# lastz/lastz

Measured on AMD Instinct MI355X. Metric: Gbp-of-target aligned/sec (whole job, --nogapped HSP path, both strands), higher is better.
Workload: dtype s32

## Files before the change

lastz_amd/csrc/lz_ctx.hpp:

```cpp
#pragma once
#include <hip/hip_runtime.h>
#include <string>
#include <vector>
#include <map>
#include <mutex>
#include "lz_common.hpp"
#include "../../include/lzgpu.h"

struct DevBuf {
    void*  p = nullptr;
    size_t cap = 0;
    int ensure(size_t bytes);
    void release();
    template <class T> T* as() const { return (T*)p; }
};

struct KernelTimer {
    struct Pending { int id; hipEvent_t a, b; hipStream_t s; };
    bool enabled = false;
    std::vector<std::string> names;
    std::vector<uint64_t> launches;
    std::vector<double> ms;
    std::vector<Pending> pending;
    std::map<hipStream_t, std::vector<hipEvent_t>> pool;
// ... 31 lines not shown
    bool inited = false;
    int  device = -1;
    int  num_cus = 256;
    hipStream_t stream = nullptr;
    hipStream_t stream2 = nullptr, stream3 = nullptr;
    hipStream_t dp_stream = nullptr;
    hipEvent_t ev_keys[LZ_SETS] = {}, ev_summ[LZ_SETS] = {}, ev_part[LZ_SETS] = {}, ev_extended[LZ_SETS] = {}, ev_init = nullptr;
    std::string last_error;

    SeqSlot target;
    bool have_table = false;
    lz_table_geom geom;
    LzSeedDev seed;
    DevBuf wstart, wpos;
    u64 num_words = 0;

    std::map<int, SeqSlot> queries;
#define LZ_TEMP_SLOT_B3 (-1000)
    std::mutex slots_m;

    DevBuf cnt, off, pk;
    DevBuf wiv, wsk, wsv;
    DevBuf blk_start;
    std::vector<u64> blk_start_host;
    u32 blk_shift = 0, blk_count = 1;
    u64* pinned = nullptr; size_t pinned_words = 0;
    DevBuf bins[LZ_SETS];
    DevBuf keys[LZ_SETS];
    DevBuf recs[LZ_SETS], bin_base[LZ_SETS];
    DevBuf hist[LZ_SETS], hist_part[LZ_SETS];
// ... 37 lines not shown
int lzk_sample_offsets(LzCtx& c, const u64* off, const u32* cnt, u32 n, u32 stride, u32 ns, u64* out);
int lzk_fill_hits(LzCtx& c, u32 lo, u32 i0, u32 i1, const u32* sk, const u32* sv, u32 n, const u64* off, u64 base, u64* keys, hipStream_t st);
int lzk_hsp_match_counts(LzCtx& c, const LzHspRec* recs, const u32* n_rec_dev, u32 cap, u32 launch_for,
                         const u8* traw, const u8* qraw, const u8* tcode, const u8* qcode, u32* counts, hipStream_t s);
struct LzLutParams; struct LzLutEntry;
#ifndef LZ_PP_TILE_HOST
#define LZ_PP_TILE_HOST 16384
#endif
int lzk_pack2(LzCtx& c, const u8* code_base, const u8* raw_base, u32 len, u8* two, u8* spc, u32 nmask, u32* flags256);
int lzk_overlap32(LzCtx& c, const u8* src, u8* dst, size_t nblocks);
int lzk_hist(LzCtx& c, const u8* bins, u64 n, u32* hist, u32* part, u32* bin_base, hipStream_t st);
int lzk_scan_reserve(LzCtx& c, int set, int mode, u64 max_n);
int lzk_scan_hits(LzCtx& c, int set, int mode, const LzExtendParams& P, const LzLutParams& Q, const u64* keys, u64 n,
                  const s32* score_tab, const LzLutEntry* lut, u8* bins, hipStream_t st);
int lzk_partition(LzCtx& c, int set, const u64* keys, u64 n, const u32* hist, const u32* part, u64* recs, hipStream_t st);
int lzk_settle(LzCtx& c, const LzExtendParams& P, const u64* recs, const u32* bin_base, u32* diag_end,
               const s32* score_tab, LzHspRec* out, u32* out_count, u32 out_cap, u64* counters, hipStream_t s);
```

lastz_amd/csrc/lz_lut.hpp:

```cpp
#pragma once
#include "lz_common.hpp"

#define LZ_PAD2         128
#define LZ_LUT_ENTRIES  4096
#define LZ_LUT_TOTAL    (2 * LZ_LUT_ENTRIES)
#define LZ_LUT_WIN_G    15
#define LZ_LUT_WIN_B    60
#define LZ_LUT_MAXWIN   3
#define LZ_GRAY(c)      ((c) ^ ((c) >> 1))

struct alignas(8) LzLutEntry { u32 ab; u32 sc; };

struct LzLutParams {
    const u8* t2; const u8* q2;
    const u8* tsp; const u8* qsp;
    const u8* t2x; const u8* tspx;
    const u8* tcode; const u8* qcode;
    s32 xdrop;
};

struct LzLutScan { u32 s; s32 run, best; u32 room, used, alive, nwin; };

#if defined(__HIP_DEVICE_COMPILE__)
LZ_HD u32 lz_alignbit(u32 hi, u32 lo, u32 sh) { return __builtin_amdgcn_alignbit(hi, lo, sh); }
// ... 187 lines not shown
{
    s32 diag; LzLutScan L, R;
    lz_lut_init(key, tlen, qlen, diag, L, R);
    while (L.alive == 1 && L.nwin < (u32)LZ_LUT_MAXWIN) lz_lut_step<false, SPECIAL>(P, lut, diag, L, ctab);
    while (R.alive == 1 && R.nwin < (u32)LZ_LUT_MAXWIN) lz_lut_step<true, SPECIAL>(P, lut, diag, R, ctab);
    return lz_lut_summary(L, R, min_score);
}

LZ_HD u64 lz_hit_record(u64 key, u32 summ)
{
    const u32 pos2 = (u32)key, diag = (u32)(key >> 32);
    const bool slow = (summ & LZ_SUMM_SLOW) != 0;
    const u64 payload = slow ? (u64)(diag >> 16) : (u64)(summ & 0xFFFFu);
    return (u64)pos2 | ((u64)(diag & 0xFFu) << 31) | (payload << 39) | (slow ? (1ull << 63) : 0ull);
}
#define LZ_REC_POS2(r)    ((u32)((r) & 0x7FFFFFFFu))
#define LZ_REC_LOW8(r)    ((u32)((r) >> 31) & 0xFFu)
#define LZ_REC_PAYLOAD(r) ((u32)((r) >> 39) & 0xFFFFu)
#define LZ_REC_SLOW(r)    ((u32)((r) >> 63))
LZ_HD u64 lz_rec_with_index(u64 r, u32 idx)
{ return (r & ~((0xFFull << 31) | (0x1Full << 55))) | ((u64)(idx & 0xFFu) << 31) | ((u64)((idx >> 8) & 0x1Fu) << 55); }
#define LZ_REC_INDEX(r)   (((u32)((r) >> 31) & 0xFFu) | (((u32)((r) >> 55) & 0x1Fu) << 8))

template <class Emit>
LZ_HD void lz_settle_record(const LzExtendParams& P, const s32* score_tab, u64 rec, u32 h ,
                            u32& dend, u64& n_ext, u64& n_bp, Emit&& emit)
{
    const u32 p2 = LZ_REC_POS2(rec);
    if (dend > p2 - P.seed_len) return;
    n_ext++;
// ... 12 lines not shown
```

lastz_amd/csrc/lzgpu_api.hip:

```cpp
#include <hip/hip_runtime.h>
#include <stdarg.h>
#include <stdio.h>
#include <stdlib.h>
#include <string.h>
#include <math.h>
#include <algorithm>
#include <mutex>
#include <thread>
#include <atomic>
#include "lz_ctx.hpp"
#include "lz_host.hpp"
#include "lz_lut.hpp"


static LzCtx g_ctx;
static void lz_release_statics();
void lz_phase_clocks_print();
LzCtx& lz_ctx() { return g_ctx; }

static thread_local std::string t_last_error, t_last_error_out;
static std::mutex g_err_m;
int lz_fail(int code, const char* fmt, ...)
{
    char buf[512];
// ... 163 lines not shown

extern "C" void lzgpu_shutdown(void)
{
    LzCtx& c = g_ctx;
    if (!c.inited) return;
    (void)hipSetDevice(c.device);
    (void)hipStreamSynchronize(c.stream);
    lz_phase_clocks_print();
    if (c.stream2) (void)hipStreamSynchronize(c.stream2);
    if (c.stream3) (void)hipStreamSynchronize(c.stream3);
    if (c.dp_stream) (void)hipStreamSynchronize(c.dp_stream);
    c.timer.resolve(); c.dp_timer.resolve();
    if (c.pinned) { (void)hipHostFree(c.pinned); c.pinned = nullptr; c.pinned_words = 0; }
    DevBuf* bufs[] = { &c.target.raw, &c.target.code, &c.wstart, &c.wpos, &c.cnt, &c.off, &c.pk, &c.wiv, &c.wsk, &c.wsv, &c.lut,
                       &c.sort_tmp, &c.scan_tmp, &c.diag_end, &c.score_tab, &c.hsp_out, &c.hsp_count, &c.hsp_mc,
                       &c.dev_counters, &c.tb_keys, &c.tb_vals, &c.tb_keys2, &c.tb_vals2 };
    for (DevBuf* b : bufs) b->release();
    for (int k = 0; k < LZ_SETS; k++) { DevBuf* sb[] = { &c.bins[k], &c.keys[k], &c.recs[k], &c.bin_base[k], &c.hist[k], &c.hist_part[k], &c.summ[k], &c.scan_tasks[k], &c.scan_ntasks[k] }; for (DevBuf* b : sb) b->release(); }
    for (auto& kv : c.queries) { kv.second.raw.release(); kv.second.code.release(); kv.second.dp.release(); kv.second.nib.release(); kv.second.two.release(); kv.second.spc.release(); kv.second.occ_dev.release(); }
    c.target.dp.release(); c.target.nib.release(); c.target.two.release(); c.target.spc.release(); c.target.occ_dev.release();
    c.target.two_x.release(); c.target.spc_x.release();
    lz_release_statics();
    c.queries.clear();
    (void)hipStreamDestroy(c.stream);
    if (c.stream2) (void)hipStreamDestroy(c.stream2);
    if (c.stream3) (void)hipStreamDestroy(c.stream3);
    if (c.dp_stream) (void)hipStreamDestroy(c.dp_stream);
    c.dp_stream = nullptr;
    for (int k = 0; k < LZ_SETS; k++) {
        hipEvent_t* ev[] = { &c.ev_keys[k], &c.ev_summ[k], &c.ev_part[k], &c.ev_extended[k] };
        for (hipEvent_t* e : ev) { if (*e) (void)hipEventDestroy(*e); *e = nullptr; }
    }
    if (c.ev_init) (void)hipEventDestroy(c.ev_init);
    c.ev_init = nullptr; c.stream2 = nullptr; c.stream3 = nullptr;
    c.stream = nullptr; c.inited = false; c.have_table = false; c.device = -1;
    c.n_owners = 1; c.owner = 0; c.last_order.clear();
}

extern "C" void lzgpu_free(void* p) { free(p); }


static int slot_upload(LzCtx& c, SeqSlot& s, const u8* bytes, u32 len, bool keep_host, hipStream_t st = nullptr)
{
    int rc;
    if (!st) st = c.stream;
    size_t total = (size_t)len + 2 * LZ_SEQ_PAD + 16;
    if ((rc = s.raw.ensure(total))) return rc;
    if ((rc = s.code.ensure(total))) return rc;
    LZ_HIP(hipMemsetAsync(s.raw.p, 0, total, st));
    LZ_HIP(hipMemsetAsync(s.code.p, LZ_CODE_INVALID, total, st));
// ... 156 lines not shown
    return rc;
}

extern "C" int lzgpu_table_geom(lz_table_geom* out)
{
    if (!g_ctx.have_table || !out) return lz_fail(LZGPU_ERR_STATE, "no position table");
    *out = g_ctx.geom; return 0;
}

extern "C" int lzgpu_table_adopt(const lz_table_geom* g)
{
    int rc = require_init(); if (rc) return rc;
    LzCtx& c = g_ctx;
    if (!g) return LZGPU_ERR_ARG;
    if ((rc = lzh_seed_to_dev(&g->seed, c.seed))) return rc;
    c.have_table = false; c.geom = *g; c.num_words = g->num_words;
    size_t total = (size_t)g->tlen + 2 * LZ_SEQ_PAD + 16;
    if ((rc = c.target.raw.ensure(total))) return rc;
    if ((rc = c.target.code.ensure(total))) return rc;
    LZ_HIP(hipMemsetAsync(c.target.raw.p, 0, total, c.stream));
    LZ_HIP(hipMemsetAsync(c.target.code.p, LZ_CODE_INVALID, total, c.stream));
    c.target.len = g->tlen; c.target.have_raw = true; c.target.code_key = 0; c.target.dp_key = 0; c.target.host.clear();
    if ((rc = c.wstart.ensure(((size_t)(1u << c.seed.weight) + 1) * 4))) return rc;
    if ((rc = c.wpos.ensure((size_t)(g->num_words ? g->num_words : 1) * 4))) return rc;
    LZ_HIP(hipStreamSynchronize(c.stream));
    return 0;
}

extern "C" int lzgpu_table_buffers(void* dev_ptr[3], uint64_t bytes[3])
{
    LzCtx& c = g_ctx;
// ... 2 lines not shown
    dev_ptr[1] = c.wstart.p;          bytes[1] = ((uint64_t)(1u << c.seed.weight) + 1) * 4;
    dev_ptr[2] = c.wpos.p;            bytes[2] = (uint64_t)c.num_words * 4;
    return 0;
}

extern "C" int lzgpu_table_commit(void)
{
    LzCtx& c = g_ctx;
    if (!c.target.have_raw || !c.wstart.p) return lz_fail(LZGPU_ERR_STATE, "no table buffers");
    { int rc = lz_bind_thread(); if (rc) return rc; }
    if (c.target.host.size() != c.geom.tlen) {
        c.target.host.resize(c.geom.tlen);
        if (c.geom.tlen) LZ_HIP(hipMemcpy(c.target.host.data(), c.target.raw_base(), c.geom.tlen, hipMemcpyDeviceToHost));
        c.target.code_key = 0; c.target.dp_key = 0;
    }
    c.have_table = true;
    return 0;
}

extern "C" int lzgpu_device_copy(void* dst, const void* src, uint64_t bytes)
{
    int rc = require_init(); if (rc) return rc;
    if (!bytes) return 0;
    LZ_HIP(hipMemcpyAsync(dst, src, bytes, hipMemcpyDeviceToDevice, g_ctx.stream));
    LZ_HIP(hipStreamSynchronize(g_ctx.stream));
    return 0;
}


#include <chrono>
struct HostProf {
    bool on; double t[16]; const char* names[16] = { nullptr }; int n = 0;
    std::chrono::steady_clock::time_point last;
    HostProf() { on = getenv("LZGPU_HOSTPROF") != nullptr; for (auto& x : t) x = 0; }
    void start() { if (on) last = std::chrono::steady_clock::now(); }
    void lap(int k, const char* name) {
        if (!on) return;
        auto now = std::chrono::steady_clock::now();
        t[k] += std::chrono::duration<double, std::milli>(now - last).count(); names[k] = name; if (k >= n) n = k + 1; last = now;
    }
    ~HostProf() { if (on) for (int k = 0; k < n; k++) if (names[k]) fprintf(stderr, "[lzgpu hostprof] %-28s %10.2f ms total\n", names[k], t[k]); }
};
static HostProf g_hp;

static int seed_search(const lz_search_args* a, lz_hsp** out, uint64_t* n_out)
{
    int rc = require_init(); if (rc) return rc;
    LzCtx& c = g_ctx;
    if (!a || !out || !n_out || !a->sub) return lz_fail(LZGPU_ERR_ARG, "null argument");
    *out = nullptr; *n_out = 0;
    if (!c.have_table) return lz_fail(LZGPU_ERR_STATE, "lzgpu_table_prepare has not been called");

    g_hp.start();
    SeqSlot* qs;
    if (a->query) {
        if (a->qlen >= 0x7FFFFFFFu) return LZGPU_NH_SIZE;
        qs = lz_query_slot(c, -1, true);
        if ((rc = slot_upload(c, *qs, a->query, a->qlen, false))) return rc;
// ... 65 lines not shown

    std::vector<LzChunk> chunks;
    hipError_t fetch_err = hipSuccess;
    auto off_at = [&](u32 i) -> u64 {
        if (i >= n) return total_hits;
        if (i % S == 0) return samp[i / S];
        u64 v = 0;
        hipError_t e = hipMemcpy(&v, c.off.as<u64>() + i, 8, hipMemcpyDeviceToHost);
        if (e != hipSuccess) fetch_err = e;
        return v;
    };
    if ((rc = lzh_plan_chunks(n, c.hit_capacity, S, off_at, chunks))) return rc;
    if (fetch_err != hipSuccess) return lz_fail(LZGPU_ERR_HIP, "prefix fetch failed: %s", hipGetErrorString(fetch_err));

    g_hp.lap(2, "chunk plan");
    u64 max_chunk = 0;
    for (auto& ch : chunks) if (ch.nh > max_chunk) max_chunk = ch.nh;
    static const bool overlap = getenv("LZGPU_OVERLAP") != nullptr && getenv("LZGPU_SERIAL") == nullptr;
    const int nsets = overlap ? (int)std::min<size_t>(chunks.size() ? chunks.size() : 1, LZ_SETS) : 1;
    if (max_chunk) {
        if ((rc = c.keys[0].ensure((size_t)max_chunk * 8))) return rc;
        if ((rc = c.bins[0].ensure((size_t)max_chunk + 64))) return rc;
        if (a->extend) {
            const size_t ntiles = (size_t)((max_chunk + LZ_PP_TILE_HOST - 1) / LZ_PP_TILE_HOST), nblocks = (ntiles + 255) / 256;
            for (int k = 0; k < nsets; k++) {
                if ((rc = c.keys[k].ensure((size_t)max_chunk * 8))) return rc;
                if ((rc = c.bins[k].ensure((size_t)max_chunk + 64))) return rc;
                if ((rc = c.recs[k].ensure((size_t)max_chunk * 8))) return rc;
                if ((rc = c.bin_base[k].ensure(257 * 4))) return rc;
                if ((rc = c.hist[k].ensure(ntiles * 256 * 4))) return rc;
                if ((rc = c.hist_part[k].ensure(nblocks * 256 * 4))) return rc;
            }
        }
    }
    const u32 out_cap = (u32)std::min<u64>(c.hsp_capacity, 0xFFFFFFF0ull);
    if (a->extend && (rc = c.hsp_out.ensure((size_t)out_cap * sizeof(LzHspRec)))) return rc;

    LzExtendParams P;
    P.tcode = c.target.code_base(); P.tlen = c.geom.tlen;
    P.qcode = qs->code_base();      P.qlen = qlen;
    P.xdrop = a->xdrop; P.min_score = a->hsp_threshold; P.seed_len = L;
    P.cls8 = lzh_small_classes(rowc, colc);
    const bool nibs = P.cls8 && c.target.have_nib && qs->have_nib;
    P.tnib = nibs ? c.target.nib.as<u8>() : nullptr; P.qnib = nibs ? qs->nib.as<u8>() : nullptr;

    LzLutParams Q;
    Q.t2 = c.target.two.as<u8>(); Q.q2 = qs->two.as<u8>(); Q.tsp = c.target.spc.as<u8>(); Q.qsp = qs->spc.as<u8>(); Q.xdrop = a->xdrop;
    Q.t2x = c.target.two_x.as<u8>(); Q.tspx = c.target.spc_x.as<u8>();
    Q.tcode = P.tcode; Q.qcode = P.qcode;
    int mode = 2;
    if (a->extend) {
        s32 M4[16];
// ... 2 lines not shown
        if (mode < c.min_scan_mode) mode = c.min_scan_mode;
        if (mode < 2) {
            static std::vector<LzLutEntry> lut_host; static s32 lut_m4[16]; static s32 lut_x = -1;
            if (lut_x != a->xdrop || memcmp(lut_m4, M4, sizeof(M4)) != 0 || !c.lut.p || lut_host.empty()) {
                lut_host.resize(LZ_LUT_TOTAL);
                lzh_lut_build(M4, a->xdrop, lut_host.data());
                if ((rc = c.lut.ensure(lut_host.size() * sizeof(LzLutEntry)))) return rc;
                memcpy(lut_m4, M4, sizeof(M4)); lut_x = a->xdrop;
                LZ_HIP(hipMemcpyAsync(c.lut.p, lut_host.data(), lut_host.size() * sizeof(LzLutEntry), hipMemcpyHostToDevice, c.stream));
                LZ_HIP(hipStreamSynchronize(c.stream));
            }
        }
    }
    c.last_scan_mode = mode;

    std::vector<lz_hsp> plain;
    if (a->extend && max_chunk) for (int k = 0; k < nsets; k++) if ((rc = lzk_scan_reserve(c, k, mode, max_chunk))) return rc;
    LZ_HIP(hipEventRecord(c.ev_init, c.stream));
    LZ_HIP(hipStreamWaitEvent(c.stream2, c.ev_init, 0));
    LZ_HIP(hipStreamWaitEvent(c.stream3, c.ev_init, 0));
    size_t ci = 0;
    const bool serial = !overlap;
    hipStream_t sF = c.stream, sS = serial ? c.stream : c.stream3, sB = serial ? c.stream : c.stream2;
    auto settle = [&](int set) -> int {
        LZ_HIP(hipStreamWaitEvent(sS, c.ev_part[set], 0));
        int r = lzk_settle(c, P, c.recs[set].as<u64>(), c.bin_base[set].as<u32>(), c.diag_end.as<u32>(), c.score_tab.as<s32>(),
                           c.hsp_out.as<LzHspRec>(), c.hsp_count.as<u32>(), out_cap, d_counters, sS);
        if (r) return r;
        LZ_HIP(hipEventRecord(c.ev_extended[set], sS));
        return 0;
    };
    int pending = -1;
    for (auto& ch : chunks) {
        const int set = (int)(ci % (size_t)nsets);
        if (!a->extend) {
            if ((rc = lzk_fill_hits(c, lo, ch.i0, ch.i1, c.wsk.as<u32>(), c.wsv.as<u32>(), n, c.off.as<u64>(), ch.base, c.keys[0].as<u64>(), sF))) return rc;
            std::vector<u64> hk(ch.nh);
            LZ_HIP(hipMemcpyAsync(hk.data(), c.keys[0].p, (size_t)ch.nh * 8, hipMemcpyDeviceToHost, c.stream));
            LZ_HIP(hipStreamSynchronize(c.stream));
            for (u64 k : hk) { u32 p2 = (u32)k; plain.push_back({ p2 + (u32)(k >> 32), p2, L, 0 }); }
            continue;
        }
        const bool reuse = ci >= (size_t)nsets;
        if (reuse && pending == set) { if ((rc = settle(pending))) return rc; pending = -1; }
        if (reuse) LZ_HIP(hipStreamWaitEvent(sF, c.ev_extended[set], 0));
        if ((rc = lzk_fill_hits(c, lo, ch.i0, ch.i1, c.wsk.as<u32>(), c.wsv.as<u32>(), n, c.off.as<u64>(), ch.base, c.keys[set].as<u64>(), sF))) return rc;
        LZ_HIP(hipEventRecord(c.ev_keys[set], sF));
        LZ_HIP(hipStreamWaitEvent(sS, c.ev_keys[set], 0));
        if ((rc = lzk_scan_hits(c, set, mode, P, Q, c.keys[set].as<u64>(), ch.nh, c.score_tab.as<s32>(), c.lut.as<LzLutEntry>(), c.bins[set].as<u8>(), sS))) return rc;
        LZ_HIP(hipEventRecord(c.ev_summ[set], sS));
        LZ_HIP(hipStreamWaitEvent(sB, c.ev_summ[set], 0));
        if ((rc = lzk_hist(c, c.bins[set].as<u8>(), ch.nh, c.hist[set].as<u32>(), c.hist_part[set].as<u32>(), c.bin_base[set].as<u32>(), sB))) return rc;
        if ((rc = lzk_partition(c, set, c.keys[set].as<u64>(), ch.nh, c.hist[set].as<u32>(), c.hist_part[set].as<u32>(), c.recs[set].as<u64>(), sB))) return rc;
        LZ_HIP(hipEventRecord(c.ev_part[set], sB));
        if (pending >= 0) { if ((rc = settle(pending))) return rc; }
        pending = set;
        ci++;
    }
    if (pending >= 0) { if ((rc = settle(pending))) return rc; }
    g_hp.lap(3, "chunk loop launches");
// ... 184 lines not shown
```

lastz_amd/csrc/seed_kernels.hip:

```cpp
#include <hip/hip_runtime.h>
#include <cstring>
#include <cstdio>
#include <rocprim/device/device_radix_sort.hpp>
#include <rocprim/device/device_scan.hpp>
#include <rocprim/iterator/transform_iterator.hpp>
#include "lz_ctx.hpp"
#include "lz_lut.hpp"
#include "lz_coop.hpp"

#define LZ_TPB 256

#if defined(LZ_NO_NT)
#define LZ_NT_LD(p_) (*(p_))
#define LZ_NT_ST(v_, p_) (*(p_) = (v_))
#else
#define LZ_NT_LD(p_) __builtin_nontemporal_load(p_)
#define LZ_NT_ST(v_, p_) __builtin_nontemporal_store((v_), (p_))
#endif
__global__ void __launch_bounds__(LZ_TPB)
k_encode(const u8* __restrict__ raw, u8* __restrict__ code, u32 len, const u8* __restrict__ cls)
{
    __shared__ u8 tab[256];
    tab[threadIdx.x] = cls[threadIdx.x];
    __syncthreads();
// ... 94 lines not shown
                                     c.tb_vals.as<u32>(), c.tb_vals2.as<u32>(), (size_t)n, 0u,
                                     (unsigned)c.seed.weight + 1u, c.stream));
    c.timer.end(c.stream);

    c.timer.begin("k_key_bounds_u32", c.stream);
    hipLaunchKernelGGL(k_key_bounds_u32, dim3((n + 1 + LZ_TPB - 1) / LZ_TPB), dim3(LZ_TPB), 0, c.stream,
                       c.tb_keys2.as<u32>(), n, nwords, c.wstart.as<u32>());
    c.timer.end(c.stream);
    LZ_HIP(hipGetLastError());

    u32 nw = 0;
    LZ_HIP(hipMemcpyAsync(&nw, c.wstart.as<u32>() + nwords, 4, hipMemcpyDeviceToHost, c.stream));
    LZ_HIP(hipStreamSynchronize(c.stream));
    c.timer.resolve();
    c.num_words = nw;
    if ((rc = c.wpos.ensure((size_t)(nw ? nw : 1) * 4))) return rc;
    LZ_HIP(hipMemcpyAsync(c.wpos.p, c.tb_vals2.p, (size_t)nw * 4, hipMemcpyDeviceToDevice, c.stream));
    LZ_HIP(hipStreamSynchronize(c.stream));
    return 0;
}

__global__ void __launch_bounds__(LZ_TPB)
k_table_export(const u32* __restrict__ wstart, const u32* __restrict__ wpos, u32 nwords,
               u32 adj_start, u32 step, u32* __restrict__ last, u32* __restrict__ prev)
{
    u32 w = blockIdx.x * LZ_TPB + threadIdx.x;
    if (w >= nwords) return;
    u32 a = wstart[w], b = wstart[w + 1];
    if (a == b) return;
    if (last) last[w] = (wpos[a] - adj_start) / step;
// ... 913 lines not shown
        else           hipLaunchKernelGGL(k_scan_tasks<1>, dim3(std::min<u32>(n_regions, 4u * (u32)cus)), dim3(LZ_ST_TPB), 0, st, P, Q, lut, score_tab, tasks, ntk, n_regions, task_cap, summ);
        c.timer.end(st);
        LZ_HIP(hipGetLastError());
    }
    return 0;
}

int lzk_partition(LzCtx& c, int set, const u64* keys, u64 n, const u32* hist, const u32* part, u64* recs, hipStream_t st)
{
    if (n == 0) return 0;
    const u32 ntiles = (u32)((n + LZ_PP_TILE - 1) / LZ_PP_TILE);
    c.timer.begin("k_partition", st);
    static const bool ballots = getenv("LZGPU_PARTITION_BALLOTS") != nullptr;
    if (ballots) hipLaunchKernelGGL(k_partition<false>, dim3(ntiles), dim3(LZ_PP_TPB), 0, st, keys, c.summ[set].as<u32>(), n, hist, part, recs);
    else         hipLaunchKernelGGL(k_partition<true>, dim3(ntiles), dim3(LZ_PP_TPB), 0, st, keys, c.summ[set].as<u32>(), n, hist, part, recs);
    c.timer.end(st);
    LZ_HIP(hipGetLastError());
    return 0;
}

__device__ __forceinline__ LzCoopMap lz_coop_shfl_up32(const LzCoopMap& v, int d)
{ LzCoopMap r; r.A = __shfl_up(v.A, d, 32); r.B = __shfl_up(v.B, d, 32); r.C = __shfl_up(v.C, d, 32); return r; }
__device__ LzCoopSide lz_coop_extend_wave(const LzExtendParams& P, const s32* tab, u32 pos1, s32 diag, s32 stopl, s32 stopr, u32 lane)
{
    const s32 X = P.xdrop;
    const bool right = lane >= 32u;
    const u32 hl = lane & 31u;
    const s32 stop = right ? stopr : stopl;
    LzCoopSide out; out.stop_pos = pos1; out.best_pos = pos1; out.best = 0;
    s32 run0 = 0, best0 = 0; u32 s = pos1;
// ... 322 lines not shown
```

Baseline: 0.3442.

## Fuse hit fill with LUT scan and tag records with bin for partition

Adds a fused kernel that expands seed hits and runs the LUT-based ungapped scan in one pass, writing tagged hit records directly instead of first materializing keys and then rescanning them. A per-word target context cache (32 bytes per word) is prebuilt so the scan can load target windows contiguously, and the bin tag is embedded in each record so histogram and partition read it without a separate bins array. The aim is to cut global memory traffic and kernel launches on the nogapped path, at the cost of extra device memory for the word context and a more complex kernel with large shared-memory use.

Result: faster. 0.3894 (median of 6 runs) (+13.1%).

```diff
diff --git a/lastz_amd/csrc/lz_ctx.hpp b/lastz_amd/csrc/lz_ctx.hpp
--- a/lastz_amd/csrc/lz_ctx.hpp
+++ b/lastz_amd/csrc/lz_ctx.hpp
@@ -69,6 +69,9 @@
     LzSeedDev seed;
     DevBuf wstart, wpos;
     u64 num_words = 0;
+    u64 table_gen = 0;
+    DevBuf wctx;
+    u64 wctx_gen = 0; uint64_t wctx_code_key = 0;
 
     std::map<int, SeqSlot> queries;
 #define LZ_TEMP_SLOT_B3 (-1000)
@@ -136,5 +139,11 @@
 int lzk_scan_hits(LzCtx& c, int set, int mode, const LzExtendParams& P, const LzLutParams& Q, const u64* keys, u64 n,
                   const s32* score_tab, const LzLutEntry* lut, u8* bins, hipStream_t st);
 int lzk_partition(LzCtx& c, int set, const u64* keys, u64 n, const u32* hist, const u32* part, u64* recs, hipStream_t st);
+int lzk_wctx_build(LzCtx& c);
+int lzk_fused_reserve(LzCtx& c, int set, u64 max_n);
+int lzk_scan_fused(LzCtx& c, int set, u32 lo, u32 i0, u32 i1, const u32* sk, const u32* sv, u32 n, const u64* off, u64 base, u64 n_hits,
+                   const LzExtendParams& P, const LzLutParams& Q, const LzLutEntry* lut, u64* tagged, hipStream_t st);
+int lzk_hist_tagged(LzCtx& c, const u64* tagged, u64 n, u32* hist, u32* part, u32* bin_base, hipStream_t st);
+int lzk_partition_tagged(LzCtx& c, const u64* tagged, u64 n, const u32* hist, const u32* part, u64* recs, hipStream_t st);
 int lzk_settle(LzCtx& c, const LzExtendParams& P, const u64* recs, const u32* bin_base, u32* diag_end,
                const s32* score_tab, LzHspRec* out, u32* out_count, u32 out_cap, u64* counters, hipStream_t s);
diff --git a/lastz_amd/csrc/lz_lut.hpp b/lastz_amd/csrc/lz_lut.hpp
--- a/lastz_amd/csrc/lz_lut.hpp
+++ b/lastz_amd/csrc/lz_lut.hpp
@@ -225,6 +225,26 @@
     const u64 payload = slow ? (u64)(diag >> 16) : (u64)(summ & 0xFFFFu);
     return (u64)pos2 | ((u64)(diag & 0xFFu) << 31) | (payload << 39) | (slow ? (1ull << 63) : 0ull);
 }
+#define LZ_REC_TAG(r)     ((u32)((r) >> 55) & 0xFFu)
+#define LZ_REC_UNTAG(r)   ((r) & ~(0xFFull << 55))
+LZ_HD u64 lz_hit_record_tagged(u64 key, u32 summ) { return lz_hit_record(key, summ) | ((u64)((u32)(key >> 40) & 0xFFu) << 55); }
+
+#define LZ_WCTX_BYTES 32
+struct alignas(16) LzWctx { u32 w[LZ_WCTX_BYTES / 4]; };
+LZ_HD u32 lz_wctx_first_byte(u32 pos1) { return ((pos1 - 1u + (u32)LZ_PAD2) >> 2) - 15u; }
+LZ_HD u32 lz_wctx_right_offset(u32 pos1) { return ((pos1 + (u32)LZ_PAD2) >> 2) - lz_wctx_first_byte(pos1); }
+LZ_HD LzWctx lz_wctx_make(const u8* two, u32 pos1) { LzWctx e; __builtin_memcpy(&e, two + lz_wctx_first_byte(pos1), LZ_WCTX_BYTES); return e; }
+LZ_HD void lz_wctx_windows(const LzWctx& e, u32 pos1, LzVec16& tl, LzVec16& tr)
+{
+    const bool at16 = lz_wctx_right_offset(pos1) == 16u;
+    LZ_UNROLL_ALL
+    for (int k = 0; k < 4; k++) {
+        tl.w[k] = e.w[k];
+        const u32 at15 = lz_alignbit(e.w[4 + k], e.w[3 + k], 24u);
+        tr.w[k] = at16 ? e.w[4 + k] : at15;
+    }
+}
+
 #define LZ_REC_POS2(r)    ((u32)((r) & 0x7FFFFFFFu))
 #define LZ_REC_LOW8(r)    ((u32)((r) >> 31) & 0xFFu)
 #define LZ_REC_PAYLOAD(r) ((u32)((r) >> 39) & 0xFFFFu)
diff --git a/lastz_amd/csrc/lzgpu_api.hip b/lastz_amd/csrc/lzgpu_api.hip
--- a/lastz_amd/csrc/lzgpu_api.hip
+++ b/lastz_amd/csrc/lzgpu_api.hip
@@ -201,7 +201,7 @@
     if (c.pinned) { (void)hipHostFree(c.pinned); c.pinned = nullptr; c.pinned_words = 0; }
     DevBuf* bufs[] = { &c.target.raw, &c.target.code, &c.wstart, &c.wpos, &c.cnt, &c.off, &c.pk, &c.wiv, &c.wsk, &c.wsv, &c.lut,
                        &c.sort_tmp, &c.scan_tmp, &c.diag_end, &c.score_tab, &c.hsp_out, &c.hsp_count, &c.hsp_mc,
-                       &c.dev_counters, &c.tb_keys, &c.tb_vals, &c.tb_keys2, &c.tb_vals2 };
+                       &c.dev_counters, &c.tb_keys, &c.tb_vals, &c.tb_keys2, &c.tb_vals2, &c.wctx };
     for (DevBuf* b : bufs) b->release();
     for (int k = 0; k < LZ_SETS; k++) { DevBuf* sb[] = { &c.bins[k], &c.keys[k], &c.recs[k], &c.bin_base[k], &c.hist[k], &c.hist_part[k], &c.summ[k], &c.scan_tasks[k], &c.scan_ntasks[k] }; for (DevBuf* b : sb) b->release(); }
     for (auto& kv : c.queries) { kv.second.raw.release(); kv.second.code.release(); kv.second.dp.release(); kv.second.nib.release(); kv.second.two.release(); kv.second.spc.release(); kv.second.occ_dev.release(); }
@@ -221,6 +221,7 @@
     if (c.ev_init) (void)hipEventDestroy(c.ev_init);
     c.ev_init = nullptr; c.stream2 = nullptr; c.stream3 = nullptr;
     c.stream = nullptr; c.inited = false; c.have_table = false; c.device = -1;
+    c.wctx_gen = 0; c.wctx_code_key = 0;
     c.n_owners = 1; c.owner = 0; c.last_order.clear();
 }
 
@@ -407,7 +408,7 @@
     LzCtx& c = g_ctx;
     if (!g) return LZGPU_ERR_ARG;
     if ((rc = lzh_seed_to_dev(&g->seed, c.seed))) return rc;
-    c.have_table = false; c.geom = *g; c.num_words = g->num_words;
+    c.have_table = false; c.geom = *g; c.num_words = g->num_words; c.table_gen++;
     size_t total = (size_t)g->tlen + 2 * LZ_SEQ_PAD + 16;
     if ((rc = c.target.raw.ensure(total))) return rc;
     if ((rc = c.target.code.ensure(total))) return rc;
@@ -440,6 +441,7 @@
         if (c.geom.tlen) LZ_HIP(hipMemcpy(c.target.host.data(), c.target.raw_base(), c.geom.tlen, hipMemcpyDeviceToHost));
         c.target.code_key = 0; c.target.dp_key = 0;
     }
+    c.table_gen++;
     c.have_table = true;
     return 0;
 }
@@ -468,6 +470,28 @@
     ~HostProf() { if (on) for (int k = 0; k < n; k++) if (names[k]) fprintf(stderr, "[lzgpu hostprof] %-28s %10.2f ms total\n", names[k], t[k]); }
 };
 static HostProf g_hp;
+
+
+static int lz_wctx_prepare(LzCtx& c, bool& fused)
+{
+    if (c.wctx.p && c.wctx_gen == c.table_gen && c.wctx_code_key == c.target.code_key && c.target.code_key) return 0;
+    const size_t need = (size_t)c.num_words * LZ_WCTX_BYTES;
+    if (c.num_words == 0) { fused = false; return 0; }
+    if (need > c.wctx.cap || !c.wctx.p) {
+        size_t fr = 0, tot = 0;
+        if (hipMemGetInfo(&fr, &tot) != hipSuccess || need > (fr + c.wctx.cap) / 2 || c.wctx.ensure(need) != 0) {
+            (void)hipGetLastError(); c.last_error.clear();
+            c.wctx_gen = 0; c.wctx_code_key = 0;
+            fused = false;
+            return 0;
+        }
+    }
+    c.wctx_gen = 0; c.wctx_code_key = 0;
+    int rc = lzk_wctx_build(c);
+    if (rc) return rc;
+    c.wctx_gen = c.table_gen; c.wctx_code_key = c.target.code_key;
+    return 0;
+}
 
 static int seed_search(const lz_search_args* a, lz_hsp** out, uint64_t* n_out)
 {
@@ -563,28 +587,6 @@
     if (fetch_err != hipSuccess) return lz_fail(LZGPU_ERR_HIP, "prefix fetch failed: %s", hipGetErrorString(fetch_err));
 
     g_hp.lap(2, "chunk plan");
-    u64 max_chunk = 0;
-    for (auto& ch : chunks) if (ch.nh > max_chunk) max_chunk = ch.nh;
-    static const bool overlap = getenv("LZGPU_OVERLAP") != nullptr && getenv("LZGPU_SERIAL") == nullptr;
-    const int nsets = overlap ? (int)std::min<size_t>(chunks.size() ? chunks.size() : 1, LZ_SETS) : 1;
-    if (max_chunk) {
-        if ((rc = c.keys[0].ensure((size_t)max_chunk * 8))) return rc;
-        if ((rc = c.bins[0].ensure((size_t)max_chunk + 64))) return rc;
-        if (a->extend) {
-            const size_t ntiles = (size_t)((max_chunk + LZ_PP_TILE_HOST - 1) / LZ_PP_TILE_HOST), nblocks = (ntiles + 255) / 256;
-            for (int k = 0; k < nsets; k++) {
-                if ((rc = c.keys[k].ensure((size_t)max_chunk * 8))) return rc;
-                if ((rc = c.bins[k].ensure((size_t)max_chunk + 64))) return rc;
-                if ((rc = c.recs[k].ensure((size_t)max_chunk * 8))) return rc;
-                if ((rc = c.bin_base[k].ensure(257 * 4))) return rc;
-                if ((rc = c.hist[k].ensure(ntiles * 256 * 4))) return rc;
-                if ((rc = c.hist_part[k].ensure(nblocks * 256 * 4))) return rc;
-            }
-        }
-    }
-    const u32 out_cap = (u32)std::min<u64>(c.hsp_capacity, 0xFFFFFFF0ull);
-    if (a->extend && (rc = c.hsp_out.ensure((size_t)out_cap * sizeof(LzHspRec)))) return rc;
-
     LzExtendParams P;
     P.tcode = c.target.code_base(); P.tlen = c.geom.tlen;
     P.qcode = qs->code_base();      P.qlen = qlen;
@@ -617,8 +619,34 @@
     }
     c.last_scan_mode = mode;
 
+    u64 max_chunk = 0;
+    for (auto& ch : chunks) if (ch.nh > max_chunk) max_chunk = ch.nh;
+    static const bool overlap = getenv("LZGPU_OVERLAP") != nullptr && getenv("LZGPU_SERIAL") == nullptr;
+    const int nsets = overlap ? (int)std::min<size_t>(chunks.size() ? chunks.size() : 1, LZ_SETS) : 1;
+    static const bool fused_off = getenv("LZGPU_FUSED_SCAN") != nullptr && atoi(getenv("LZGPU_FUSED_SCAN")) == 0;
+    bool fused = a->extend && mode == 0 && max_chunk && !fused_off && c.n_owners <= 1 && getenv("LZGPU_FILL_SHUFFLE") == nullptr;
+    if (fused && (rc = lz_wctx_prepare(c, fused))) return rc;
+    if (max_chunk) {
+        if ((rc = c.keys[0].ensure((size_t)max_chunk * 8))) return rc;
+        if (!fused && (rc = c.bins[0].ensure((size_t)max_chunk + 64))) return rc;
+        if (a->extend) {
+            const size_t ntiles = (size_t)((max_chunk + LZ_PP_TILE_HOST - 1) / LZ_PP_TILE_HOST), nblocks = (ntiles + 255) / 256;
+            for (int k = 0; k < nsets; k++) {
+                if ((rc = c.keys[k].ensure((size_t)max_chunk * 8))) return rc;
+                if (!fused && (rc = c.bins[k].ensure((size_t)max_chunk + 64))) return rc;
+                if ((rc = c.recs[k].ensure((size_t)max_chunk * 8))) return rc;
+                if ((rc = c.bin_base[k].ensure(257 * 4))) return rc;
+                if ((rc = c.hist[k].ensure(ntiles * 256 * 4))) return rc;
+                if ((rc = c.hist_part[k].ensure(nblocks * 256 * 4))) return rc;
+            }
+        }
+    }
+    const u32 out_cap = (u32)std::min<u64>(c.hsp_capacity, 0xFFFFFFF0ull);
+    if (a->extend && (rc = c.hsp_out.ensure((size_t)out_cap * sizeof(LzHspRec)))) return rc;
+
+
     std::vector<lz_hsp> plain;
-    if (a->extend && max_chunk) for (int k = 0; k < nsets; k++) if ((rc = lzk_scan_reserve(c, k, mode, max_chunk))) return rc;
+    if (a->extend && max_chunk) for (int k = 0; k < nsets; k++) if ((rc = fused ? lzk_fused_reserve(c, k, max_chunk) : lzk_scan_reserve(c, k, mode, max_chunk))) return rc;
     LZ_HIP(hipEventRecord(c.ev_init, c.stream));
     LZ_HIP(hipStreamWaitEvent(c.stream2, c.ev_init, 0));
     LZ_HIP(hipStreamWaitEvent(c.stream3, c.ev_init, 0));
@@ -647,6 +675,21 @@
         const bool reuse = ci >= (size_t)nsets;
         if (reuse && pending == set) { if ((rc = settle(pending))) return rc; pending = -1; }
         if (reuse) LZ_HIP(hipStreamWaitEvent(sF, c.ev_extended[set], 0));
+        if (fused) {
+            LZ_HIP(hipEventRecord(c.ev_keys[set], sF));
+            LZ_HIP(hipStreamWaitEvent(sS, c.ev_keys[set], 0));
+            if ((rc = lzk_scan_fused(c, set, lo, ch.i0, ch.i1, c.wsk.as<u32>(), c.wsv.as<u32>(), n, c.off.as<u64>(), ch.base, ch.nh, P, Q,
+                                     c.lut.as<LzLutEntry>(), c.keys[set].as<u64>(), sS))) return rc;
+            LZ_HIP(hipEventRecord(c.ev_summ[set], sS));
+            LZ_HIP(hipStreamWaitEvent(sB, c.ev_summ[set], 0));
+            if ((rc = lzk_hist_tagged(c, c.keys[set].as<u64>(), ch.nh, c.hist[set].as<u32>(), c.hist_part[set].as<u32>(), c.bin_base[set].as<u32>(), sB))) return rc;
+            if ((rc = lzk_partition_tagged(c, c.keys[set].as<u64>(), ch.nh, c.hist[set].as<u32>(), c.hist_part[set].as<u32>(), c.recs[set].as<u64>(), sB))) return rc;
+            LZ_HIP(hipEventRecord(c.ev_part[set], sB));
+            if (pending >= 0) { if ((rc = settle(pending))) return rc; }
+            pending = set;
+            ci++;
+            continue;
+        }
         if ((rc = lzk_fill_hits(c, lo, ch.i0, ch.i1, c.wsk.as<u32>(), c.wsv.as<u32>(), n, c.off.as<u64>(), ch.base, c.keys[set].as<u64>(), sF))) return rc;
         LZ_HIP(hipEventRecord(c.ev_keys[set], sF));
         LZ_HIP(hipStreamWaitEvent(sS, c.ev_keys[set], 0));
diff --git a/lastz_amd/csrc/seed_kernels.hip b/lastz_amd/csrc/seed_kernels.hip
--- a/lastz_amd/csrc/seed_kernels.hip
+++ b/lastz_amd/csrc/seed_kernels.hip
@@ -132,6 +132,7 @@
     LZ_HIP(hipStreamSynchronize(c.stream));
     c.timer.resolve();
     c.num_words = nw;
+    c.table_gen++;
     if ((rc = c.wpos.ensure((size_t)(nw ? nw : 1) * 4))) return rc;
     LZ_HIP(hipMemcpyAsync(c.wpos.p, c.tb_vals2.p, (size_t)nw * 4, hipMemcpyDeviceToDevice, c.stream));
     LZ_HIP(hipStreamSynchronize(c.stream));
@@ -1075,6 +1076,334 @@
     static const bool ballots = getenv("LZGPU_PARTITION_BALLOTS") != nullptr;
     if (ballots) hipLaunchKernelGGL(k_partition<false>, dim3(ntiles), dim3(LZ_PP_TPB), 0, st, keys, c.summ[set].as<u32>(), n, hist, part, recs);
     else         hipLaunchKernelGGL(k_partition<true>, dim3(ntiles), dim3(LZ_PP_TPB), 0, st, keys, c.summ[set].as<u32>(), n, hist, part, recs);
+    c.timer.end(st);
+    LZ_HIP(hipGetLastError());
+    return 0;
+}
+
+__global__ void __launch_bounds__(LZ_TPB)
+k_build_wctx(const u32* __restrict__ wpos, u64 num_words, const u8* __restrict__ two, LzVec16* __restrict__ wctx)
+{
+    const u64 j = (u64)blockIdx.x * LZ_TPB + threadIdx.x;
+    if (j >= 2 * num_words) return;
+    const u32 pos1 = wpos[j >> 1];
+    wctx[j] = lz_load16(two + lz_wctx_first_byte(pos1) + 16u * (u32)(j & 1u));
+}
+
+template <int CAP> struct LzFuse2Wave {
+    alignas(16) u32 own32[CAP / 2];
+    u32 lsrc[64 * LZ_FILL_GROUP];
+    uint2 ent[64];
+};
+struct LzFuseTrip { u32 p1, pos2, dst; bool ok; LzWctx cx; LzVec16 ql, qr; };
+
+template <bool SELF, int TPB, int CAP>
+__global__ void __launch_bounds__(TPB)
+k_scan_hits2(u32 lo, u32 i0, u32 i1, LzSeedDev sd,
+             const u32* __restrict__ wstart, const u32* __restrict__ wpos, const LzWctx* __restrict__ wctx,
+             const u32* __restrict__ sk, const u32* __restrict__ sv, u32 n, const u64* __restrict__ off, u64 base,
+             LzExtendParams P, LzLutParams Q, const LzLutEntry* __restrict__ lut_g,
+             u64* __restrict__ recs, LzScanTask* __restrict__ tasks, u32* __restrict__ n_tasks, u32 region_cap, LzSelfDev self)
+{
+    static_assert(CAP % 512 == 0, "whole 16-byte groups of own[] per lane");
+    constexpr int WORDS = CAP / 2 / 64;
+    __shared__ LzLutEntry lut[LZ_LUT_TOTAL];
+    __shared__ LzFuse2Wave<CAP> shw[TPB / 64];
+    for (u32 k = threadIdx.x; k < LZ_LUT_TOTAL; k += TPB) lut[k] = lut_g[k];
+    __syncthreads();
+    LzFuse2Wave<CAP>& sh = shw[threadIdx.x >> 6];
+    unsigned short* const own = reinterpret_cast<unsigned short*>(sh.own32);
+    const u32 lane = threadIdx.x & 63u;
+    const u32 region = blockIdx.x * (TPB / 64) + (threadIdx.x >> 6), nwaves = gridDim.x * (TPB / 64);
+    LzScanTask* const my_tasks = tasks + (size_t)region * region_cap;
+    u32 my_n = 0;
+    const u32 ngroups = (n + 63u) / 64u;
+    for (u32 grp = region; grp < ngroups; grp += nwaves) {
+        const u32 j = grp * 64u + lane;
+        u32 w_l = 0, i_l = 0; bool in = false;
+        if (j < n) { w_l = sk[j] & ((2u << sd.weight) - 1u); i_l = sv[j]; in = !(w_l >> sd.weight) && i_l >= i0 && i_l < i1; }
+        if (!__ballot(in)) continue;
+        const u32 dbase = in ? (u32)(off[i_l] - base) : 0u;
+        const u32 pos2 = lo + i_l + 1u;
+        u32 slo = 0, shi = 0;
+        if (SELF) lz_self_bounds(self, pos2, slo, shi);
+        u32 carry = 0;
+        for (int r = 0; r < sd.nprobes; r += LZ_FILL_GROUP) {
+            u32 la[LZ_FILL_GROUP], len[LZ_FILL_GROUP]; u32 total = 0;
+#pragma unroll
+            for (int p = 0; p < LZ_FILL_GROUP; p++) {
+                const bool on = in && r + p < sd.nprobes;
+                const u32 w = on ? (w_l ^ sd.probe_xor[(r + p) & (LZ_MAX_PROBES - 1)]) : 0u;
+                la[p] = wstart[w]; len[p] = wstart[w + 1];
+            }
+#pragma unroll
+            for (int p = 0; p < LZ_FILL_GROUP; p++) {
+                const bool on = in && r + p < sd.nprobes;
+                len[p] = on ? len[p] - la[p] : 0u;
+                if (!SELF) total += len[p];
+            }
+            if (SELF) {
+                lz_clip_runs<LZ_FILL_GROUP>(wpos, la, len, slo, shi);
+#pragma unroll
+                for (int p = 0; p < LZ_FILL_GROUP; p++) total += len[p];
+            }
+            u32 inc = total;
+            LZ_WAVE_SCAN_U32(inc, total, lz_uadd)
+            const u32 E = inc - total;
+            const u32 T = (u32)__builtin_amdgcn_readlane((int)inc, 63);
+            {
+                u32 S = E;
+#pragma unroll
+                for (int p = 0; p < LZ_FILL_GROUP; p++) { sh.lsrc[lane * LZ_FILL_GROUP + p] = la[p] - S; S += len[p]; }
+            }
+            sh.ent[lane] = make_uint2(dbase + carry - E, pos2);
+            for (u32 cs = 0; cs < T; cs += CAP) {
+                const u32 tc = (T - cs < (u32)CAP) ? T - cs : (u32)CAP;
+                uint4* const mine = reinterpret_cast<uint4*>(sh.own32 + lane * WORDS);
+#pragma unroll
+                for (int k = 0; k < WORDS / 4; k++) mine[k] = make_uint4(0u, 0u, 0u, 0u);
+                __atomic_signal_fence(__ATOMIC_SEQ_CST);
+                {
+                    u32 S = E;
+#pragma unroll
+                    for (int p = 0; p < LZ_FILL_GROUP; p++) {
+                        const u32 l = len[p];
+                        if (l && S < cs + tc && S + l > cs) own[(S > cs ? S : cs) - cs] = (unsigned short)(1u + lane * LZ_FILL_GROUP + (u32)p);
+                        S += l;
+                    }
+                }
+                __atomic_signal_fence(__ATOMIC_SEQ_CST);
+                u32 wv[WORDS];
+#pragma unroll
+                for (int k = 0; k < WORDS / 4; k++) { const uint4 v = mine[k]; wv[4 * k] = v.x; wv[4 * k + 1] = v.y; wv[4 * k + 2] = v.z; wv[4 * k + 3] = v.w; }
+                u32 segmax = 0;
+#pragma unroll
+                for (int k = 0; k < WORDS; k++) { const u32 m2 = lz_umax(wv[k] & 0xFFFFu, wv[k] >> 16); segmax = lz_umax(segmax, m2); }
+                u32 sinc = segmax;
+                LZ_WAVE_SCAN_U32(sinc, segmax, lz_umax)
+                u32 run = lz_dpp_u32<0x138, 0xf, 0xf>(0u, sinc);
+#pragma unroll
+                for (int k = 0; k < WORDS; k++) {
+                    const u32 a0 = lz_umax(wv[k] & 0xFFFFu, run), a1 = lz_umax(wv[k] >> 16, a0);
+                    wv[k] = a0 | (a1 << 16); run = a1;
+                }
+#pragma unroll
+                for (int k = 0; k < WORDS / 4; k++) mine[k] = make_uint4(wv[4 * k], wv[4 * k + 1], wv[4 * k + 2], wv[4 * k + 3]);
+                __atomic_signal_fence(__ATOMIC_SEQ_CST);
+                auto load_trip = [&](u32 tb, LzFuseTrip& t) {
+                    const u32 t0 = tb + lane;
+                    t.ok = t0 < tc;
+                    const u32 tt = t.ok ? t0 : tc - 1u;
+                    const u32 list = (u32)own[tt] - 1u;
+                    const u32 ls = sh.lsrc[list];
+                    const uint2 en = sh.ent[list / LZ_FILL_GROUP];
+                    const u32 tabs = cs + tt, e = ls + tabs;
+                    t.p1 = wpos[e]; t.cx = wctx[e];
+                    t.pos2 = en.y; t.dst = en.x + tabs;
+                    const u32 sql = en.y - 1u + (u32)LZ_PAD2;
+                    t.ql = lz_load16(Q.q2 + ((sql >> 2) - 15u)); t.qr = lz_load16(Q.q2 + ((sql + 1u) >> 2));
+                };
+                auto scan_trip = [&](const LzFuseTrip& t) {
+                    const u64 key = lz_hit_key(t.p1, t.pos2);
+                    LzLutRaw<false> rl, rr;
+                    lz_wctx_windows(t.cx, t.p1, rl.tv, rr.tv);
+                    rl.qv = t.ql; rr.qv = t.qr;
+                    u32 summ;
+                    lz_scan_round<false>(P, Q, lut, nullptr, key, t.ok, rl, rr, t.dst, lane, summ, my_tasks, my_n, region_cap);
+                    if (t.ok) LZ_NT_ST(lz_hit_record_tagged(key, summ), recs + t.dst);
+                };
+                LzFuseTrip ta, tb2;
+                load_trip(0u, ta);
+#pragma unroll 1
+                for (u32 tb = 0;;) {
+                    if (tb + 64u < tc) load_trip(tb + 64u, tb2);
+                    scan_trip(ta);
+                    tb += 64u; if (tb >= tc) break;
+                    if (tb + 64u < tc) load_trip(tb + 64u, ta);
+                    scan_trip(tb2);
+                    tb += 64u; if (tb >= tc) break;
+                }
+                __atomic_signal_fence(__ATOMIC_SEQ_CST);
+            }
+            carry += total;
+        }
+    }
+    if (lane == 0) n_tasks[region] = my_n < region_cap ? my_n : region_cap;
+}
+
+__global__ void __launch_bounds__(LZ_ST_TPB)
+k_scan_tasks2(LzExtendParams P, LzLutParams Q, const LzLutEntry* __restrict__ lut_g, const LzScanTask* __restrict__ tasks,
+              const u32* __restrict__ n_tasks, u32 n_regions, u32 region_cap, u64* __restrict__ recs)
+{
+    __shared__ LzLutEntry lut[LZ_LUT_TOTAL];
+    for (u32 k = threadIdx.x; k < LZ_LUT_TOTAL; k += LZ_ST_TPB) lut[k] = lut_g[k];
+    __syncthreads();
+    for (u32 region = blockIdx.x; region < n_regions; region += gridDim.x) {
+        const u32 nt = n_tasks[region];
+        for (u32 k = threadIdx.x; k < nt; k += (u32)LZ_ST_TPB) {
+            const LzScanTask t = tasks[(size_t)region * region_cap + k];
+            LzLutScan L = t.L, R = t.R;
+            const u32 pos1 = L.alive == 1 ? L.s + (u32)LZ_LUT_WIN_B * L.nwin : R.s - (u32)LZ_LUT_WIN_B * R.nwin;
+            while (L.alive == 1 && L.nwin < (u32)LZ_LUT_MAXWIN) lz_lut_step<false, false>(Q, lut, t.diag, L, nullptr);
+            while (R.alive == 1 && R.nwin < (u32)LZ_LUT_MAXWIN) lz_lut_step<true, false>(Q, lut, t.diag, R, nullptr);
+            recs[t.idx] = lz_hit_record_tagged(lz_hit_key(pos1, pos1 - (u32)t.diag), lz_lut_summary(L, R, P.min_score));
+        }
+    }
+}
+
+__global__ void __launch_bounds__(LZ_TPB)
+k_hist2(const u64* __restrict__ tagged, u64 n, u32* __restrict__ hist)
+{
+    __shared__ u32 cnt[LZ_NBIN];
+    cnt[threadIdx.x] = 0;
+    __syncthreads();
+    const u64 base = (u64)blockIdx.x * LZ_PP_TILE;
+    typedef u64 lz_u64x2 __attribute__((ext_vector_type(2)));
+#pragma unroll 4
+    for (int r = 0; r < LZ_PP_TILE / (LZ_TPB * 2); r++) {
+        const u64 i = base + ((u64)r * LZ_TPB + threadIdx.x) * 2u;
+        if (i + 1u < n) {
+            const lz_u64x2 v = *reinterpret_cast<const lz_u64x2*>(tagged + i);
+            atomicAdd(&cnt[LZ_REC_TAG(v.x)], 1u); atomicAdd(&cnt[LZ_REC_TAG(v.y)], 1u);
+        } else if (i < n) atomicAdd(&cnt[LZ_REC_TAG(tagged[i])], 1u);
+    }
+    __syncthreads();
+    hist[(size_t)blockIdx.x * LZ_NBIN + threadIdx.x] = cnt[threadIdx.x];
+}
+
+__global__ void __launch_bounds__(LZ_PP_TPB)
+k_partition2(const u64* __restrict__ tagged, u64 n, const u32* __restrict__ hist, const u32* __restrict__ part, u64* __restrict__ recs)
+{
+    __shared__ LzPartShared sh;
+    const u32 tid = threadIdx.x, lane = tid & 63u, w = tid >> 6;
+    const u32 tile = blockIdx.x;
+    const u64 base = (u64)tile * LZ_PP_TILE;
+    const u32 tile_n = (n - base < (u64)LZ_PP_TILE) ? (u32)(n - base) : (u32)LZ_PP_TILE;
+    for (u32 k = tid; k < LZ_PP_WAVES * LZ_NBIN; k += LZ_PP_TPB) { (&sh.wcnt[0][0])[k] = 0; (&sh.bm[0][0])[k] = 0ull; }
+    const u32 l0 = w * (64u * LZ_PP_ROUNDS) + lane;
+    u64 rr[LZ_PP_ROUNDS];
+#pragma unroll
+    for (u32 r = 0; r < LZ_PP_ROUNDS; r++) rr[r] = (l0 + 64u * r < tile_n) ? tagged[base + l0 + 64u * r] : 0ull;
+    __syncthreads();
+    u32 slot[LZ_PP_ROUNDS];
+#pragma unroll
+    for (u32 r = 0; r < LZ_PP_ROUNDS; r++) {
+        const bool valid = l0 + 64u * r < tile_n;
+        const u32 bin = LZ_REC_TAG(rr[r]);
+        if (valid) atomicOr((unsigned long long*)&sh.bm[w][bin], 1ull << lane);
+        const u64 peers = valid ? sh.bm[w][bin] : 0ull;
+        const u32 old = valid ? sh.wcnt[w][bin] : 0u;
+        if (valid && (peers >> lane) == 1ull) { sh.wcnt[w][bin] = old + (u32)__popcll(peers); sh.bm[w][bin] = 0ull; }
+        slot[r] = old + (u32)__popcll(peers & ((1ull << lane) - 1ull));
+    }
+    __syncthreads();
+    u32 tot = 0;
+    if (tid < LZ_NBIN) {
+        for (u32 k = 0; k < LZ_PP_WAVES; k++) { const u32 v = sh.wcnt[k][tid]; sh.wcnt[k][tid] = tot; tot += v; }
+        sh.gbase[tid] = part[(size_t)(tile >> 8) * LZ_NBIN + tid] + hist[(size_t)tile * LZ_NBIN + tid];
+    }
+    const u32 ts = lz_exscan256(tot, sh.wtot);
+    if (tid < LZ_NBIN) sh.tstart[tid] = ts;
+    if (tid == 0) sh.tstart[LZ_NBIN] = tile_n;
+    __syncthreads();
+#pragma unroll
+    for (u32 r = 0; r < LZ_PP_ROUNDS; r++) {
+        const u32 bin = LZ_REC_TAG(rr[r]);
+        if (l0 + 64u * r < tile_n) sh.stage[sh.tstart[bin] + sh.wcnt[w][bin] + slot[r]] = rr[r];
+    }
+    __syncthreads();
+    for (u32 k = tid; k < tile_n; k += LZ_PP_TPB) {
+        const u64 r = sh.stage[k];
+        const u32 b = LZ_REC_TAG(r);
+        recs[(size_t)sh.gbase[b] + (k - sh.tstart[b])] = LZ_REC_UNTAG(r);
+    }
+}
+
+int lzk_wctx_build(LzCtx& c)
+{
+    const u64 nw = c.num_words;
+    if (nw == 0) return 0;
+    c.timer.begin("k_build_wctx", c.stream);
+    hipLaunchKernelGGL(k_build_wctx, dim3((unsigned)((2 * nw + LZ_TPB - 1) / LZ_TPB)), dim3(LZ_TPB), 0, c.stream,
+                       c.wpos.as<u32>(), nw, c.target.two.as<u8>(), c.wctx.as<LzVec16>());
+    c.timer.end(c.stream);
+    LZ_HIP(hipGetLastError());
+    return 0;
+}
+
+static u32 lz_fused_tpb(LzCtx& c)
+{
+    static const int env = getenv("LZGPU_FUSE_TPB") ? atoi(getenv("LZGPU_FUSE_TPB")) : 0;
+    if (c.self.mode != LZ_SELF_OFF) return 512u;
+    return (env == 512 || env == 768 || env == 1024) ? (u32)env : 1024u;
+}
+static void lz_fused_geometry(LzCtx& c, u64 n_hits, u32& grid, u32& n_regions, u32& region_cap)
+{
+    int cus = 256; (void)hipDeviceGetAttribute(&cus, hipDeviceAttributeMultiprocessorCount, c.device);
+    grid = (u32)cus; n_regions = grid * (lz_fused_tpb(c) / 64u);
+    region_cap = (u32)std::min<u64>(n_hits / 32 / n_regions + 64, 1u << 20);
+    static const char* force = getenv("LZGPU_TASK_REGION_CAP");
+    if (force && atoi(force) > 0) region_cap = (u32)atoi(force);
+}
+int lzk_fused_reserve(LzCtx& c, int set, u64 max_n)
+{
+    u32 grid, n_regions, region_cap; int rc;
+    lz_fused_geometry(c, max_n, grid, n_regions, region_cap);
+    if ((rc = c.scan_tasks[set].ensure((size_t)n_regions * region_cap * sizeof(LzScanTask)))) return rc;
+    return c.scan_ntasks[set].ensure((size_t)n_regions * 4);
+}
+int lzk_scan_fused(LzCtx& c, int set, u32 lo, u32 i0, u32 i1, const u32* sk, const u32* sv, u32 n, const u64* off, u64 base, u64 n_hits,
+                   const LzExtendParams& P, const LzLutParams& Q, const LzLutEntry* lut, u64* tagged, hipStream_t st)
+{
+    if (n == 0 || i1 <= i0 || n_hits == 0) return 0;
+    if (!c.blk_start_host.empty()) {
+        const u32 b0 = i0 >> c.blk_shift, b1 = (i1 - 1) >> c.blk_shift;
+        const u64 j0 = c.blk_start_host[b0], j1 = c.blk_start_host[std::min<u32>(b1 + 1, c.blk_count)];
+        sk += j0; sv += j0; n = (u32)(j1 - j0);
+        if (n == 0) return 0;
+    }
+    int rc;
+    u32 grid, n_regions, region_cap;
+    lz_fused_geometry(c, n_hits, grid, n_regions, region_cap);
+    if ((rc = c.scan_tasks[set].ensure((size_t)n_regions * region_cap * sizeof(LzScanTask)))) return rc;
+    if ((rc = c.scan_ntasks[set].ensure((size_t)n_regions * 4))) return rc;
+    LzScanTask* tasks = c.scan_tasks[set].as<LzScanTask>(); u32* ntk = c.scan_ntasks[set].as<u32>();
+    c.timer.begin("k_scan_hits", st);
+    const u32 tpb = lz_fused_tpb(c);
+#define LZ_FUSED_LAUNCH(S_, T_, C_, self_) hipLaunchKernelGGL((k_scan_hits2<S_, T_, C_>), dim3(grid), dim3(T_), 0, st, lo, i0, i1, c.seed, c.wstart.as<u32>(), c.wpos.as<u32>(), \
+                           c.wctx.as<LzWctx>(), sk, sv, n, off, base, P, Q, lut, tagged, tasks, ntk, region_cap, self_)
+    if (c.self.mode != LZ_SELF_OFF) LZ_FUSED_LAUNCH(true, 512, 2560, c.self);
+    else if (tpb == 512)            LZ_FUSED_LAUNCH(false, 512, 2560, LzSelfDev{});
+    else if (tpb == 768)            LZ_FUSED_LAUNCH(false, 768, 1024, LzSelfDev{});
+    else                            LZ_FUSED_LAUNCH(false, 1024, 512, LzSelfDev{});
+#undef LZ_FUSED_LAUNCH
+    c.timer.end(st);
+    LZ_HIP(hipGetLastError());
+    c.timer.begin("k_scan_tasks", st);
+    hipLaunchKernelGGL(k_scan_tasks2, dim3(std::min<u32>(n_regions, 4u * grid)), dim3(LZ_ST_TPB), 0, st, P, Q, lut, tasks, ntk, n_regions, region_cap, tagged);
+    c.timer.end(st);
+    LZ_HIP(hipGetLastError());
+    return 0;
+}
+int lzk_hist_tagged(LzCtx& c, const u64* tagged, u64 n, u32* hist, u32* part, u32* bin_base, hipStream_t st)
+{
+    const u32 ntiles = (u32)((n + LZ_PP_TILE - 1) / LZ_PP_TILE), nblocks = (ntiles + 255u) / 256u;
+    c.timer.begin("k_hist", st);
+    hipLaunchKernelGGL(k_hist2, dim3(ntiles), dim3(LZ_TPB), 0, st, tagged, n, hist);
+    c.timer.end(st);
+    c.timer.begin("k_hist_scan", st);
+    hipLaunchKernelGGL(k_hist_scan1, dim3(nblocks), dim3(LZ_NBIN), 0, st, hist, ntiles, part);
+    hipLaunchKernelGGL(k_hist_scan2, dim3(1), dim3(LZ_NBIN), 0, st, part, nblocks, bin_base);
+    c.timer.end(st);
+    LZ_HIP(hipGetLastError());
+    return 0;
+}
+int lzk_partition_tagged(LzCtx& c, const u64* tagged, u64 n, const u32* hist, const u32* part, u64* recs, hipStream_t st)
+{
+    if (n == 0) return 0;
+    const u32 ntiles = (u32)((n + LZ_PP_TILE - 1) / LZ_PP_TILE);
+    c.timer.begin("k_partition", st);
+    hipLaunchKernelGGL(k_partition2, dim3(ntiles), dim3(LZ_PP_TPB), 0, st, tagged, n, hist, part, recs);
     c.timer.end(st);
     LZ_HIP(hipGetLastError());
     return 0;
```
